# ailabspace/drl-based-mapless-crowd-navigation-with-perceived-risk

Measured on AMD Instinct MI355X. Metric: env-steps/sec @4096 envs×20 peds×360 rays; HBM GB/s vs roofline, higher is better.
Workload: dtype f64

## Files before the change

### drl-based-mapless-crowd-navigation-with-perceived-risk_amd/csrc/crowdnav_device.h

```cpp
#pragma once
#include <hip/hip_runtime.h>
#include <stdint.h>

#define CN_PI 3.14159265358979323846

typedef const __attribute__((address_space(4))) int32_t* cn_kflag;

__device__ __forceinline__ double cn_round_scaled(double x, double p, cn_kflag py2)
{
    double y = x * p;
    double r = rint(y);
    double d = y - r;
    const bool tie = fabs(d) == 0.5;
    unsigned long long any_tie = __builtin_amdgcn_ballot_w64(tie);
    asm("" : "+s"(any_tie));
    if (__builtin_expect(any_tie != 0ull, 0)) {
        if (tie) {
            double err = fma(x, p, -y);
            if (err > 0.0) r = y + 0.5;
            else if (err < 0.0) r = y - 0.5;
            else if (*py2) r = y + copysign(0.5, y);
        }
    }
    return r;
}
__device__ __forceinline__ double cn_py_round(double x, double p, cn_kflag py2) { return cn_round_scaled(x, p, py2) / p; }
__device__ __forceinline__ double cn_np_around(double x, double p) { return rint(x * p) / p; }

#define CN_INV1000 (1.0 / 1000.0)
#define CN_INV100 (1.0 / 100.0)
__device__ __forceinline__ double cn_div1000(double r)
{
    double q = r * CN_INV1000;
    return fma(fma(-q, 1000.0, r), CN_INV1000, q);
}
__device__ __forceinline__ double cn_div100(double r)
{
    double q = r * CN_INV100;
    return fma(fma(-q, 100.0, r), CN_INV100, q);
}
__device__ __forceinline__ double cn_py_round3(double x, cn_kflag py2)
{
    double r = cn_round_scaled(x, 1000.0, py2);
    return (fabs(r) < 2147483648.0) ? cn_div1000(r) : r / 1000.0;
}
__device__ __forceinline__ double cn_py_round2(double x, cn_kflag py2)
{
    double r = cn_round_scaled(x, 100.0, py2);
    return (fabs(r) < 2147483648.0) ? cn_div100(r) : r / 100.0;
}
__device__ __forceinline__ double cn_np_around3(double x)
{
    double r = rint(x * 1000.0);
    return (fabs(r) < 2147483648.0) ? cn_div1000(r) : r / 1000.0;
}
template <bool SMALL> __device__ __forceinline__ double cn_py_round3_t(double x, cn_kflag py2)
{
    if constexpr (SMALL) return cn_div1000(cn_round_scaled(x, 1000.0, py2)); else return cn_py_round3(x, py2);
}
template <bool SMALL> __device__ __forceinline__ double cn_np_around3_t(double x)
{
    if constexpr (SMALL) return cn_div1000(rint(x * 1000.0)); else return cn_np_around3(x);
}
__device__ __forceinline__ double cn_np_around2(double x)
{
    double r = rint(x * 100.0);
    return (fabs(r) < 2147483648.0) ? cn_div100(r) : r / 100.0;
}
template <bool SMALL> __device__ __forceinline__ double cn_py_round2_t(double x, cn_kflag py2)
{
    if constexpr (SMALL) return cn_div100(cn_round_scaled(x, 100.0, py2)); else return cn_py_round2(x, py2);
}
template <bool SMALL> __device__ __forceinline__ double cn_np_around2_t(double x)
{
    if constexpr (SMALL) return cn_div100(rint(x * 100.0)); else return cn_np_around2(x);
}
template <bool SMALL> __device__ __forceinline__ double cn_round_np64_2_t(double x, cn_kflag py2)
{
    const double y = x * 100.0;
    double r = rint(y);
    if (__builtin_expect(fabs(y - r) == 0.5, 0) && *py2) r = cn_round_scaled(x, 100.0, py2);
    if constexpr (SMALL) return cn_div100(r); else return (fabs(r) < 2147483648.0) ? cn_div100(r) : r / 100.0;
}

__host__ __device__ inline void cn_det_sincos(double x, double* sn, double* cs)
{
    const double two_over_pi = 6.36619772367581382433e-01;
    const double p1 = 1.57079632673412561417e+00;
    const double p2 = 6.07710050630396597660e-11;
    const double p3 = 2.02226624879595063154e-21;
    double fn = rint(x * two_over_pi);
    double r = fma(-fn, p1, x);
    r = fma(-fn, p2, r);
    r = fma(-fn, p3, r);
    double z = r * r;
    const double S1 = -1.66666666666666324348e-01, S2 = 8.33333333332248946124e-03,
                 S3 = -1.98412698298579493134e-04, S4 = 2.75573137070700676789e-06,
                 S5 = -2.50507602534068634195e-08, S6 = 1.58969099521155010221e-10;
    double ps = fma(z, S6, S5);
    ps = fma(z, ps, S4);
    ps = fma(z, ps, S3);
    ps = fma(z, ps, S2);
    ps = fma(z, ps, S1);
    double s = fma(r * z, ps, r);
    const double C1 = 4.16666666666666019037e-02, C2 = -1.38888888888741095749e-03,
                 C3 = 2.48015872894767294178e-05, C4 = -2.75573143513906633035e-07,
                 C5 = 2.08757232129817482790e-09, C6 = -1.13596475577881948265e-11;
// ... 178 lines not shown
}

__host__ __device__ inline uint64_t cn_mix64(uint64_t z)
{
    z += 0x9E3779B97F4A7C15ULL;
    z = (z ^ (z >> 30)) * 0xBF58476D1CE4E5B9ULL;
    z = (z ^ (z >> 27)) * 0x94D049BB133111EBULL;
    return z ^ (z >> 31);
}
__host__ __device__ inline double cn_rng_u01(uint64_t seed, int64_t env, uint32_t stream, uint32_t a, uint32_t b)
{
    uint64_t h = cn_mix64(seed ^ cn_mix64((uint64_t)env));
    h = cn_mix64(h ^ (((uint64_t)stream << 32) | (uint64_t)a));
    h = cn_mix64(h ^ (uint64_t)b);
    return (double)(h >> 11) * (1.0 / 9007199254740992.0);
}

__host__ __device__ inline double cn_clamp(double x, double lo, double hi) { return fmin(fmax(x, lo), hi); }

__device__ __forceinline__ double cn_iou3(double ax, double ay, double bx, double by, double half, cn_kflag py2)
{
    double axp = ax + half, axm = ax - half, ayp = ay + half, aym = ay - half;
    double bxp = bx + half, bxm = bx - half, byp = by + half, bym = by - half;
    double ix = cn_vmin(axp, bxp) - cn_vmax(axm, bxm);
    double iy = cn_vmin(ayp, byp) - cn_vmax(aym, bym);
    if (!(ix > 0.0 && iy > 0.0)) return 0.0;
    double inter = ix * iy;
    double area_a = (axp - axm) * (ayp - aym);
    double area_b = (bxp - bxm) * (byp - bym);
    double uni = area_a + area_b - inter;
    return cn_py_round3(inter / uni, py2);
}

__device__ __forceinline__ bool cn_iou3_positive(double ax, double ay, double bx, double by, double half, cn_kflag py2)
{
    double axp = ax + half, axm = ax - half, ayp = ay + half, aym = ay - half;
    double bxp = bx + half, bxm = bx - half, byp = by + half, bym = by - half;
    double ix = cn_vmin(axp, bxp) - cn_vmax(axm, bxm);
    double iy = cn_vmin(ayp, byp) - cn_vmax(aym, bym);
    if (!(ix > 0.0 && iy > 0.0)) return false;
    double inter = ix * iy;
    double area_a = (axp - axm) * (ayp - aym);
    double area_b = (bxp - bxm) * (byp - bym);
    double uni = area_a + area_b - inter;
    if (inter > 0.00075 * uni) return true;
    return cn_py_round3(inter / uni, py2) > 0.0;
}

__device__ __forceinline__ double cn_shfl_xor_d(double v, int m)
{
    int lo = __double2loint(v), hi = __double2hiint(v);
    lo = __shfl_xor(lo, m, 64);
    hi = __shfl_xor(hi, m, 64);
    return __hiloint2double(hi, lo);
}
template <int CTRL, int ROW_MASK>
__device__ __forceinline__ int cn_dpp_i(int ident, int v) { return __builtin_amdgcn_update_dpp(ident, v, CTRL, ROW_MASK, 0xf, false); }
template <int CTRL, int ROW_MASK>
__device__ __forceinline__ double cn_dpp_d(double ident, double v)
{
    int lo = __builtin_amdgcn_update_dpp(__double2loint(ident), __double2loint(v), CTRL, ROW_MASK, 0xf, false);
    int hi = __builtin_amdgcn_update_dpp(__double2hiint(ident), __double2hiint(v), CTRL, ROW_MASK, 0xf, false);
    return __hiloint2double(hi, lo);
}
template <int N> __device__ __forceinline__ int cn_row_shr_i(int ident, int v) { static_assert(N >= 1 && N <= 15, "row_shr"); return cn_dpp_i<0x110 + N, 0xf>(ident, v); }
template <int N> __device__ __forceinline__ int cn_row_shl_i(int ident, int v) { static_assert(N >= 1 && N <= 15, "row_shl"); return cn_dpp_i<0x100 + N, 0xf>(ident, v); }
#pragma clang diagnostic push
#pragma clang diagnostic ignored "-Winline-asm"
__device__ __forceinline__ unsigned long long cn_writelane_u64(unsigned long long v, unsigned long long x, int l)
{
    unsigned lo = (unsigned)v, hi = (unsigned)(v >> 32);
    const unsigned xl = __builtin_amdgcn_readfirstlane((unsigned)x), xh = __builtin_amdgcn_readfirstlane((unsigned)(x >> 32));
    const int ls = __builtin_amdgcn_readfirstlane(l);
    asm("s_mov_b32 m0, %4\n\tv_writelane_b32 %0, %2, m0\n\tv_writelane_b32 %1, %3, m0"
        : "+v"(lo), "+v"(hi) : "s"(xl), "s"(xh), "s"(ls) : "m0");
    return ((unsigned long long)hi << 32) | lo;
}
#pragma clang diagnostic pop
__device__ __forceinline__ unsigned long long cn_readlane_u64(unsigned long long v, int l)
{
    const unsigned lo = (unsigned)__builtin_amdgcn_readlane((int)(unsigned)v, l), hi = (unsigned)__builtin_amdgcn_readlane((int)(unsigned)(v >> 32), l);
    return ((unsigned long long)hi << 32) | lo;
}
#define CN_DPP_REDUCE(T, DPP, v, ident, OP)                         \
    do {                                                            \
        v = OP(v, DPP<0x111, 0xf>(ident, v));        \
        v = OP(v, DPP<0x112, 0xf>(ident, v));        \
        v = OP(v, DPP<0x114, 0xf>(ident, v));        \
        v = OP(v, DPP<0x118, 0xf>(ident, v));        \
        v = OP(v, DPP<0x142, 0xa>(ident, v));     \
        v = OP(v, DPP<0x143, 0xc>(ident, v));     \
    } while (0)
__device__ __forceinline__ double cn_lane63_d(double v)
{
    int lo = __builtin_amdgcn_readlane(__double2loint(v), 63), hi = __builtin_amdgcn_readlane(__double2hiint(v), 63);
    return __hiloint2double(hi, lo);
}
__device__ __forceinline__ double cn_wave_min_d(double v)
{
    const double id = INFINITY;
    CN_DPP_REDUCE(double, cn_dpp_d, v, id, cn_vmin);
    return cn_lane63_d(v);
}
__device__ __forceinline__ double cn_wave_max_d(double v)
{
    const double id = -INFINITY;
    CN_DPP_REDUCE(double, cn_dpp_d, v, id, cn_vmax);
    return cn_lane63_d(v);
}
__device__ __forceinline__ int cn_add_i(int a, int b) { return a + b; }
__device__ __forceinline__ int cn_wave_min_i(int v)
{
    const int id = 0x7fffffff;
    CN_DPP_REDUCE(int, cn_dpp_i, v, id, min);
    return __builtin_amdgcn_readlane(v, 63);
}
__device__ __forceinline__ int cn_wave_max_i(int v)
{
    const int id = (int)0x80000000;
    CN_DPP_REDUCE(int, cn_dpp_i, v, id, max);
    return __builtin_amdgcn_readlane(v, 63);
}
__device__ __forceinline__ int cn_wave_sum_i(int v)
{
    const int id = 0;
    CN_DPP_REDUCE(int, cn_dpp_i, v, id, cn_add_i);
    return __builtin_amdgcn_readlane(v, 63);
}
```

### drl-based-mapless-crowd-navigation-with-perceived-risk_amd/csrc/crowdnav_kernel.hip

```cpp
#include "crowdnav_device.h"
#include "crowdnav_kernel.h"

#define CN_SYNC() do { __builtin_amdgcn_fence(__ATOMIC_RELEASE, "wavefront"); __builtin_amdgcn_wave_barrier(); \
                       __builtin_amdgcn_fence(__ATOMIC_ACQUIRE, "wavefront"); } while (0)

__device__ __forceinline__ void cn_setprio_uniform(int v)
{
    if (v == 0) __builtin_amdgcn_s_setprio(0); else if (v == 1) __builtin_amdgcn_s_setprio(1);
    else if (v == 2) __builtin_amdgcn_s_setprio(2); else __builtin_amdgcn_s_setprio(3);
}
#define CN_FAIR_AT(k) do { if constexpr (FAIR) { if ((k) == 0) __builtin_amdgcn_s_setprio(3); else if ((k) == 7) __builtin_amdgcn_s_setprio(2); \
                           else if ((k) == 11) __builtin_amdgcn_s_setprio(1); else if ((k) == 15) __builtin_amdgcn_s_setprio(0); } \
                           else if constexpr (SFENCE) { if ((k) == 0 || (k) == 7 || (k) == 11 || (k) == 15) __builtin_amdgcn_s_setprio(0); } } while (0)
#ifdef CN_TIMING
#define CN_ABLATE(bit) (p->ablate & (bit))
#define CN_T(k) do { CN_FAIR_AT(k); if (p->timing && lane == 0) p->timing[(size_t)env * 32 + (k)] = (long long)__builtin_amdgcn_s_memtime(); \
                     if (((p->ablate >> 8) & 0xff) == (k) + 1 && (!((p->ablate >> 16) & 1) || (env & 3) != 0)) __builtin_amdgcn_endpgm(); } while (0)
#else
#define CN_ABLATE(bit) 0
#define CN_T(k) CN_FAIR_AT(k)
#endif

#define CN_XBAR() do { asm volatile("s_waitcnt lgkmcnt(0)\n\ts_barrier" ::: "memory"); } while (0)
struct XMail { double px, py, sy, cy, ox, oy, smin1, pad; int nnear, wall_x, wall_y, nocc, fast_assoc, k1, fe1, lb1, ns1; };
// ... 976 lines not shown
        for (int j = lane; j < nconf; j += 64) chk_set<CMP>(L, j, 0);
        CN_SYNC();
        if (nconf == 0) {
            e.ntracks = 0;
        } else {
            unsigned long long alive = 0ull;
            int cur = nt0;
            int mybj = 0; bool mymatch = false;
            for (int t0 = 0; t0 < nt0; t0 += 8) {
                const int ti = t0 + (lane >> 3);
                double best = -1.0; int bj = 0x7fffffff;
                if (ti < nt0) {
                    const double tx = TRK(CN_TF_PX, ti), ty_ = TRK(CN_TF_PY, ti);
                    for (int oj = lane & 7; oj < nconf; oj += 8) {
                        const double u = cn_iou3(tx, ty_, cfx_at<CMP>(L, oj), cfy_at<CMP>(L, oj), 0.0505, PY2);
                        if (u > best) { best = u; bj = oj; }
                    }
                }
#define CN_AM_STEP(CTRL) { const double ob = cn_dpp_d<CTRL, 0xf>(best, best); const int ojx = cn_dpp_i<CTRL, 0xf>(bj, bj); \
                           if (ob > best || (ob == best && ojx < bj)) { best = ob; bj = ojx; } }
                CN_AM_STEP(0xF5)
                CN_AM_STEP(0xEE)
                CN_AM_STEP(0x104)
#undef CN_AM_STEP
                const u64 posm = __ballot(best > 0.0);
                const int wb = __shfl(bj, (lane & 7) * 8, 64);
                if ((lane >> 3) == (t0 >> 3)) { mybj = wb; mymatch = ((posm >> (8 * (lane & 7))) & 1ull) != 0ull; }
            }
            const u64 matchm = __ballot(mymatch && lane < nt0);
            for (int i = 0; i < nt0; ++i) {
                if ((matchm >> i) & 1ull) alive |= (1ull << i);
                else if (cur > i) cur -= 1;
                else alive |= (1ull << i);
            }
            if (lane < nt0 && ((matchm >> lane) & 1ull)) {
                const int i = lane;
                double cxj = cfx_at<CMP>(L, mybj), cyj = cfy_at<CMP>(L, mybj);
                TRK(CN_TF_PX, i) = cxj; TRK(CN_TF_PY, i) = cyj; TRK(CN_TF_DIST, i) = cfd_at<CMP>(L, mybj);
                if (TRK(CN_TF_DQLEN, i) < 1.5) { TRK(CN_TF_D1X, i) = cxj; TRK(CN_TF_D1Y, i) = cyj; TRK(CN_TF_DQLEN, i) = 2.0; }
                TRK(CN_TF_T, i) = now - TRK(CN_TF_T, i);
                chk_set<CMP>(L, mybj, 1);
            }
            CN_SYNC();
            double rec[CN_TF_COUNT];
            bool mine = (lane < nt0) && ((alive >> lane) & 1ull);
            if (mine) {
#pragma unroll
                for (int f = 0; f < CN_TF_COUNT; ++f) rec[f] = TRK(f, lane);
            }
            CN_SYNC();
            if (mine) {
                int slot = __popcll(alive & ((1ull << lane) - 1ull));
#pragma unroll
                for (int f = 0; f < CN_TF_COUNT; ++f) TRK(f, slot) = rec[f];
            }
            e.ntracks = __popcll(alive);
            add_unchecked = true;
        }
    }
    CN_SYNC();
    if (add_unchecked) {
        for (int j0 = 0; j0 < nconf; j0 += 64) {
            int j = j0 + lane;
            bool want = (j < nconf) && !chk_at<CMP>(L, j) && (cft_at<CMP>(L, j) == TY_O);
            unsigned long long m = __ballot(want);
            int slot = e.ntracks + __popcll(m & ((1ull << lane) - 1ull));
            if (want) {
                if (slot < L.tcap) {
                    double cxj = cfx_at<CMP>(L, j), cyj = cfy_at<CMP>(L, j);
                    TRK(CN_TF_PX, slot) = cxj; TRK(CN_TF_PY, slot) = cyj; TRK(CN_TF_DIST, slot) = cfd_at<CMP>(L, j);
                    TRK(CN_TF_D0X, slot) = cxj; TRK(CN_TF_D0Y, slot) = cyj; TRK(CN_TF_D1X, slot) = 0.0; TRK(CN_TF_D1Y, slot) = 0.0;
                    TRK(CN_TF_T, slot) = now; TRK(CN_TF_SPEED, slot) = -1.0;
                    TRK(CN_TF_VX, slot) = 0.0; TRK(CN_TF_VY, slot) = 0.0; TRK(CN_TF_DQLEN, slot) = 1.0;
                }
            }
            int total = e.ntracks + __popcll(m);
            if (total > L.tcap) { e.status |= CN_ST_TRACK_OVERFLOW; total = L.tcap; }
            e.ntracks = total;
        }
    }
    CN_SYNC();
}

template <bool EXT, bool GT = false, bool FAIR = false, bool CMP = false, bool X2 = false, bool SF = false, bool HOIST = true, bool WIDE = false>
__device__ __forceinline__ void observe(KP p, const Poly& pg, EnvRegs& e, const Lds& L, int env, int lane, int step_counter,
                        float* obs32, float* fin32, double* obs64, int* done_out, bool have_tg = false, Trig tg = Trig{0.0, 0.0, 0.0, 0.0},
                        const int wv = 0, XMail* const mb = nullptr)
{
    constexpr bool SFENCE = SF || (CMP && !FAIR);
    static_assert(!X2 || (!EXT && !GT), "two wavefronts per environment: simulated sensors, lidar-tracker mode");
    static_assert(!WIDE || (!GT && !CMP && !X2), "the wide tracker table: lidar-tracker mode, plain layout, one wavefront");
    const bool w0 = !X2 || wv == 0;
    const int R = p->R, n = R - 1, K = p->K, D = n + 7 + 4 * K;
    const double MAXR = p->max_scan_range;
    double px = e.rx, py = e.ry;
    const double yaw = e.ryaw, v = e.rv, w = e.rw, now = e.clock;
    double distance_to_goal = 0.0, heading = 0.0, agent_vel_x = 0.0, agent_vel_y = 0.0;
    double sy = 0.0, cy = 0.0, ox = 0.0, oy = 0.0;
    const double h = p->room_half;
    int nnear = 0;
    u64 blkw = 0ull;
    bool wall_x = false, wall_y = false;
    if (w0) {
    CN_T(22);
    if (step_counter == 1) waypoint_refresh(p, pg, e, lane, px, py);
    distance_to_goal = cn_round_np64_2_t<!EXT>(dist3(px, py, e.wpx, e.wpy), PY2);
    heading = cn_py_round2_t<!EXT>(heading_to_goal(p, e, px, py, yaw), PY2);
    CN_T(23);
    if (step_counter % 5 == 0 || distance_to_goal < e.prev_dist) waypoint_refresh(p, pg, e, lane, px, py);
    CN_T(24);
    double sw_, cw_;
    if (have_tg) { sw_ = tg.sw; cw_ = tg.cw; } else cn_det_sincos_t(p->trig, w, &sw_, &cw_);
    agent_vel_x = -1.0 * (v * cw_);
    agent_vel_y = v * sw_;

    CN_T(2);
    if (have_tg) { sy = tg.sy; cy = tg.cy; } else cn_det_sincos_t(p->trig, yaw, &sy, &cy);
    ox = fma(p->lidar_offset_x, cy, px); oy = fma(p->lidar_offset_x, sy, py);
    if constexpr (X2) { if (lane == 0) { mb->px = px; mb->py = py; mb->sy = sy; mb->cy = cy; mb->ox = ox; mb->oy = oy; } }
    }
    if constexpr (X2) CN_XBAR();
    if (w0) {
    nnear = near_peds(p, L, lane, ox, oy, sy, cy, X2 ? nullptr : &blkw);
    wall_x = !(h - fabs(ox) > p->lidar_max + 1e-6);
    wall_y = !(h - fabs(oy) > p->lidar_max + 1e-6);
    if constexpr (X2) { if (lane == 0) { mb->nnear = nnear; mb->wall_x = wall_x; mb->wall_y = wall_y; } }
    }
    if constexpr (X2) {
        CN_XBAR();
        if (!w0) {
            px = mb->px; py = mb->py; sy = mb->sy; cy = mb->cy; ox = mb->ox; oy = mb->oy;
            nnear = mb->nnear; wall_x = mb->wall_x != 0; wall_y = mb->wall_y != 0;
        }
    }
    CN_T(3);
    double smin = 1e300;
    float* o32 = obs32 + (size_t)env * D;
    float* f32 = fin32 ? fin32 + (size_t)env * D : nullptr;
    double* o64 = obs64 ? obs64 + (size_t)env * D : nullptr;
    const double* const lidc = p->lidar_c; const double* const lids = p->lidar_s;
    const double* const angs = p->ang_s; const double* const angc = p->ang_c;
    short assoc_pre = 0;
    if (!GT && p->assoc_fast && lane <= p->assoc_k1 + 1) assoc_pre = p->assoc_tab[lane];
    double lmin_reg = 0.0;
    int rare_reg = 0;
    if constexpr (HOIST) {
        lmin_reg = p->lidar_min;
        rare_reg = (p->scan_f32 != 0 ? 1 : 0) | (p->lidar_min_positive ? 0 : 2);
        asm volatile("" : "+v"(lmin_reg), "+v"(rare_reg));
    }
    for (int k = X2 ? lane + 64 * wv : lane; k < R; k += X2 ? 128 : 64) {
        double lc = 0.0, ls = 0.0, tS = 0.0, tC = 0.0;
        if (!EXT) { lc = cn_ldg(lidc, (unsigned)k); ls = cn_ldg(lids, (unsigned)k); }
        if (!GT) { tS = cn_ldg(angs, (unsigned)(R - 1 - k)); tC = cn_ldg(angc, (unsigned)(R - 1 - k)); }
        const double t = cast_ray<EXT>(p, L, env, k, ox, oy, sy, cy, nnear, wall_x, wall_y, lc, ls, X2 ? nullptr : &blkw, HOIST ? &lmin_reg : nullptr, HOIST);
        if (k >= 1) {
            const unsigned j = (unsigned)(R - 1 - k);
            double r = t;
            double sc;
            if constexpr (EXT) {
                if (isinf(r) && r > 0) sc = MAXR;
                else if (r != r) sc = 0.0;
                else if (r == 0.0) sc = MAXR;
                else if (r > MAXR) sc = MAXR;
                else sc = r;
            } else {
                sc = cn_vmin(r, MAXR);
                const int rare = HOIST ? __builtin_amdgcn_readfirstlane(rare_reg) : (p->lidar_min_positive ? 0 : 2);
                if (__builtin_expect(rare != 0, 0)) {
                    if (rare & 1) r = (double)(float)r;
                    sc = cn_vmin(r, MAXR);
                    if ((rare & 2) && r == 0.0) sc = MAXR;
                }
            }
            smin = cn_vmin(smin, sc);
            if constexpr (!GT) {
            const double sa = fma(tS, cy, -(tC * sy)), ca = fma(tC, cy, tS * sy);
            pt_set<CMP>(L, j, (int)cn_round_scaled(px + (sc * ca), 1000.0, PY2), (int)cn_round_scaled(py + (sc * sa) * -1.0, 1000.0, PY2));
            L.dmil[j] = (unsigned short)(int)cn_round_scaled(sc, 1000.0, PY2);
            }
            double so = cn_np_around3_t<!EXT>(sc);
            cn_stg(o32, j, (float)so);
            if (f32) cn_stg(f32, j, (float)so);
            if (o64) cn_stg(o64, j, so);
        }
    }
    CN_T(4);
    bool too_close = __ballot(smin < p->min_scan_range) != 0ull;
    CN_SYNC();
    if constexpr (X2) {
        if (!w0 && lane == 0) mb->smin1 = too_close ? -1.0 : 1e300;
        CN_XBAR();
        if (w0) too_close = too_close || (mb->smin1 < 0.0);
    }

    if (w0 && step_counter == 0) {
        if (!EXT && p->bb_spawn_valid && px == p->spawn_x && py == p->spawn_y && yaw == p->spawn_yaw) e.bb = p->bb_spawn;
        else e.bb = bbox_size(p, L.stage, lane, n, px, py, yaw);
        double qx = cn_py_round3_t<!EXT>(px, PY2), qy = cn_py_round3_t<!EXT>(py, PY2);
        if (e.dq_len < 2) { if (e.dq_len == 0) { e.dq0x = qx; e.dq0y = qy; } else { e.dq1x = qx; e.dq1y = qy; } e.dq_len += 1; }
        else { e.dq0x = e.dq1x; e.dq0y = e.dq1y; e.dq1x = qx; e.dq1y = qy; }
    }

    CN_T(5);
    int ego_hit = 0;
    double* const T = WIDE ? L.gtrk : L.trk;
    double* const CPV = WIDE ? L.gcpv : L.cpv;
    if constexpr (!GT) {
    const int W = (n + 63) >> 6;
#define WORD(id, q) L.w64[__mul24((id), L.wstride) + (q)]
#define BIT(id, i) ((WORD(id, (i) >> 6) >> ((i) & 63)) & 1ull)
#define PX(i) cn_div1000((double)ptx_at<CMP>(L, (i)))
#define PY(i) cn_div1000((double)pty_at<CMP>(L, (i)))
#define GNONE 0x7fffffff
    unsigned short* occlist = L.srcidx;
    int nocc = 0;
    u64 occraw = 0ull;
    if (w0)
    for (int q = 0; q < W; ++q) {
        const int i = lane + 64 * q;
        const bool oc = (i < n) && (L.dmil[i] != 600);
        if (i < n) L.gq[i] = GNONE;
        const u64 bo = __ballot(oc);
        if (oc) occlist[nocc + __popcll(bo & ((1ull << lane) - 1ull))] = (unsigned short)i;
        occraw = cn_writelane_u64(occraw, bo, q);
        nocc += __popcll(bo);
    }
    if (w0 && lane < W) { WORD(M_NONE, lane) = ~0ull; WORD(M_ZERO, lane) = 0ull; WORD(M_EQ, lane) = 0ull; WORD(M_NNONE, lane) = 0ull; WORD(M_NZERO, lane) = 0ull; }
    CN_SYNC();
    if constexpr (X2) {
        if (w0 && lane == 0) mb->nocc = nocc;
        CN_XBAR();
        if (!w0) nocc = mb->nocc;
    }
    for (int c0 = 0; c0 < nocc; c0 += 128) {
        const int ca = X2 ? c0 + 64 * wv + lane : c0 + lane, cb = X2 ? nocc : ca + 64;
        const bool two = !X2 && c0 + 64 < nocc;
        const bool va = ca < nocc, vb = cb < nocc;
        const int ia = va ? (int)occlist[ca] : 0, ib = vb ? (int)occlist[cb] : 0;
        const int ja = (ia == n - 1) ? 0 : ia + 1, jb = (ib == n - 1) ? 0 : ib + 1;
        const int xai = ptx_at<CMP>(L, ia), yai = pty_at<CMP>(L, ia), xaj = ptx_at<CMP>(L, ja), yaj = pty_at<CMP>(L, ja);
        int xbi = 0, ybi = 0, xbj = 0, ybj = 0;
        if (two) { xbi = ptx_at<CMP>(L, ib); ybi = pty_at<CMP>(L, ib); xbj = ptx_at<CMP>(L, jb); ybj = pty_at<CMP>(L, jb); }
        const double dya = cn_div1000((double)yai) - cn_div1000((double)yaj);
        const double qa = (dya == 0) ? 0.0 : cn_div(cn_div1000((double)xai) - cn_div1000((double)xaj), dya);
        if (va) L.gq[ia] = (int)cn_round_scaled(qa, 1000.0, PY2);
        if (two) {
            const double dyb = cn_div1000((double)ybi) - cn_div1000((double)ybj);
            const double qb = (dyb == 0) ? 0.0 : cn_div(cn_div1000((double)xbi) - cn_div1000((double)xbj), dyb);
            if (vb) L.gq[ib] = (int)cn_round_scaled(qb, 1000.0, PY2);
        }
    }
    int lastnn = -1;
    if (nocc > 0) {
        lastnn = occlist[nocc - 1];
        if (lastnn == n - 1) lastnn = (nocc > 1) ? (int)occlist[nocc - 2] : -1;
    }
    CN_SYNC();
    if constexpr (X2) CN_XBAR();
#define CHG(a_, b_) (((a_) == GNONE || (b_) == GNONE) ? CN_NAN : fabs(cn_div1000((double)(a_)) - cn_div1000((double)(b_))))
    double clast = CN_NAN;
    if (L.gq[n - 1] != GNONE && lastnn >= 0) clast = CHG(L.gq[lastnn], L.gq[lastnn + 1]);
// ... 356 lines not shown
#undef GNONE
    e.nconf = nconf;
    CN_SYNC();

    int n_obst = 0;
    for (int j = lane; j < nconf; j += 64) {
        if (cft_at<CMP>(L, j) == TY_O) { n_obst += 1; if (cfd_at<CMP>(L, j) < 0.140) ego_hit = 1; }
    }
    n_obst = cn_wave_sum_i(n_obst);
    ego_hit = cn_wave_max_i(ego_hit);
    if (n_obst > 0) e.obst_steps += 1;

    CN_T(13);
    if constexpr (WIDE) tracker_stage_wide(p, e, L, T, lane, nconf, now);
    else tracker_stage<CMP>(p, e, L, T, lane, nconf, now);
    } else {
        const int P_ = p->P;
        const double r_ = p->ped_radius, lim_ = p->lidar_max + r_, lim2_ = lim_ * lim_;
        int nt_ = 0;
        u64 hitm = 0ull;
        for (int i0 = 0; i0 < P_; i0 += 64) {
            const int i = i0 + lane;
            bool inr = false, seg = false, blocked = false;
            double cx = 0.0, cyy = 0.0, wx = 0.0, wy = 0.0, len2 = 0.0;
            if (i < P_) {
                cx = L.ped[2 * i]; cyy = L.ped[2 * i + 1];
                const double ocx = cx - ox, ocy = cyy - oy;
                const double dd2 = fma(ocx, ocx, ocy * ocy);
                inr = dd2 <= lim2_;
                if (inr) {
                    const double dd = cn_sqrt(dd2);
                    if (dd > r_) {
                        seg = true;
                        const double k_ = (dd - r_) / dd;
                        wx = k_ * ocx; wy = k_ * ocy;
                        len2 = fma(wx, wx, wy * wy);
                    }
                }
            }
            for (int j0 = 0; j0 < P_; j0 += 64) {
                const int jl = j0 + lane;
                bool jin = false;
                if (jl < P_) { const double qx = L.ped[2 * jl] - ox, qy = L.ped[2 * jl + 1] - oy; jin = fma(qx, qx, qy * qy) <= lim2_; }
                u64 jm = __ballot(jin);
                while (jm) {
                    const int j = j0 + __builtin_ctzll(jm);
                    jm &= jm - 1ull;
                    const double qx = L.ped[2 * j] - ox, qy = L.ped[2 * j + 1] - oy;
                    if (seg && j != i) {
                        double tau = (len2 > 0.0) ? fma(qx, wx, qy * wy) / len2 : 0.0;
                        tau = fmin(fmax(tau, 0.0), 1.0);
                        const double ex = fma(tau, wx, -qx), ey = fma(tau, wy, -qy);
                        if (fma(ex, ex, ey * ey) < r_ * r_) blocked = true;
                    }
                }
            }
            const bool vis = inr && !blocked;
            const u64 vm = __ballot(vis);
            const int slot = nt_ + __popcll(vm & ((1ull << lane) - 1ull));
            bool close_ = false;
            if (vis && slot < L.tcap) {
                const double dx = cx - px, dy = cyy - py;
                const double dp = cn_sqrt(fma(dx, dx, dy * dy));
                double sx_ = cx, sy_ = cyy;
                if (dp > 0.0) { sx_ = cx - r_ * (dx / dp); sy_ = cyy - r_ * (dy / dp); }
                const double dist = cn_py_round3(dp - r_, PY2);
                const double vx = L.pedv[2 * i], vy = L.pedv[2 * i + 1];
                TRK(CN_TF_PX, slot) = cn_py_round3(sx_, PY2); TRK(CN_TF_PY, slot) = cn_py_round3(sy_, PY2); TRK(CN_TF_DIST, slot) = dist;
                TRK(CN_TF_D0X, slot) = 0.0; TRK(CN_TF_D0Y, slot) = 0.0; TRK(CN_TF_D1X, slot) = 0.0; TRK(CN_TF_D1Y, slot) = 0.0;
                TRK(CN_TF_T, slot) = (double)i; TRK(CN_TF_SPEED, slot) = cn_sqrt(fma(vx, vx, vy * vy));
                TRK(CN_TF_VX, slot) = -vx; TRK(CN_TF_VY, slot) = -vy; TRK(CN_TF_DQLEN, slot) = 0.0;
                close_ = dist < 0.140;
            }
            hitm |= __ballot(close_);
            nt_ += __popcll(vm);
        }
        if (nt_ > L.tcap) { e.status |= CN_ST_TRACK_OVERFLOW; nt_ = L.tcap; }
        e.ntracks = nt_; e.nconf = nt_;
        if (nt_ > 0) e.obst_steps += 1;
        ego_hit = hitm != 0ull;
        CN_SYNC();
    }
    CN_T(14);
    if constexpr (WIDE) {
        for (int it = lane; it < e.ntracks; it += 64) {
            if (TRK(CN_TF_DQLEN, it) > 1.5) {
                double dc = cn_hypot(TRK(CN_TF_D0Y, it) - TRK(CN_TF_D1Y, it), TRK(CN_TF_D0X, it) - TRK(CN_TF_D1X, it));
                TRK(CN_TF_SPEED, it) = cn_div_z(dc, TRK(CN_TF_T, it));
            }
        }
    } else
    if (lane < e.ntracks && TRK(CN_TF_DQLEN, lane) > 1.5) {
        double dc = cn_hypot(TRK(CN_TF_D0Y, lane) - TRK(CN_TF_D1Y, lane), TRK(CN_TF_D0X, lane) - TRK(CN_TF_D1X, lane));
        TRK(CN_TF_SPEED, lane) = cn_div_z(dc, TRK(CN_TF_T, lane));
    }
    CN_TSYNC();

    for (int i = lane; i < 4 * K; i += 64) {
        int c = i & 3;
        L.tail[7 + i] = (c == 0) ? px : (c == 1 ? py : 0.0);
    }
    if (lane < K) L.kidx[lane] = -1;
    e.nent = 0;
    CN_SYNC();

    CN_T(15);
    if (e.dq_len == 2 && !(CN_ABLATE(8))) {
        const double ts = e.ts;
        if (ts == 0.0) e.status |= CN_ST_DT_ZERO;
        const int nt = e.ntracks;
        double vx_ = cn_div_z(e.dq1x - e.dq0x, ts), vy_ = cn_div_z(e.dq1y - e.dq0y, ts);
        double agent_vel = cn_sqrt(vx_ * vx_ + vy_ * vy_);
        double obstacle_vel = (nt == 0) ? 0.0 : TRK(CN_TF_SPEED, 0);
        if constexpr (WIDE) {
            for (int it = lane; it < nt; it += 64)
                if (TRK(CN_TF_DQLEN, it) > 1.5) {
                    double chx = TRK(CN_TF_D0X, it) - TRK(CN_TF_D1X, it), chy = TRK(CN_TF_D0Y, it) - TRK(CN_TF_D1Y, it);
                    TRK(CN_TF_VX, it) = cn_div_z(chx, ts); TRK(CN_TF_VY, it) = cn_div_z(chy, ts);
                }
            CN_WIDE_SYNC();
        } else
        if (!GT && lane < nt && TRK(CN_TF_DQLEN, lane) > 1.5) {
            double chx = TRK(CN_TF_D0X, lane) - TRK(CN_TF_D1X, lane), chy = TRK(CN_TF_D0Y, lane) - TRK(CN_TF_D1Y, lane);
            TRK(CN_TF_VX, lane) = cn_div_z(chx, ts); TRK(CN_TF_VY, lane) = cn_div_z(chy, ts);
        }
        double vo_x = e.dq1x, vo_y = e.dq1y;
        if (nt > 0) {
            int l = nt - 1;
            double chx = 0.0, chy = 0.0;
            if (GT) { chx = TRK(CN_TF_VX, l) * ts; chy = TRK(CN_TF_VY, l) * ts; }
            else if (TRK(CN_TF_DQLEN, l) > 1.5) { chx = TRK(CN_TF_D0X, l) - TRK(CN_TF_D1X, l); chy = TRK(CN_TF_D0Y, l) - TRK(CN_TF_D1Y, l); }
            vo_x = e.dq1x + chx; vo_y = e.dq1y + chy;
        }
        CN_SYNC();
        const double a0x = e.dq0x, a0y = e.dq0y;
        double gradient = (vo_y == 0.0) ? 0.0 : cn_div(vo_x - a0x, vo_y) - a0y;
        double bb0 = a0x - (gradient * a0y);
        int hi = (int)ceil(a0x + 3.5), lo = (int)floor(a0x - 3.5);
        double ego_max = 0.0;
        const double rv = agent_vel - obstacle_vel;
        const int hcap = min(p->max_conf, 64);
        double* const hitp = L.cfx;
        for (int c0 = 0; c0 < nt; c0 += hcap) {
            const int c1 = min(nt, c0 + hcap);
            u64 nearm = 0, hasm = 0;
            for (int i = c0; i < c1; ++i) {
                const int r_ = i - c0;
                if ((r_ & 7) == 0) {
                    const int ti = i + (lane >> 3), x2l = hi - (lane & 7);
                    bool nearc = false;
                    if (ti < c1 && x2l > lo) {
                        const double ctx = TRK(CN_TF_PX, ti), cty = TRK(CN_TF_PY, ti);
                        const double y2l = ((double)x2l * gradient) + bb0;
                        const double ex = (double)x2l - a0x, ey = y2l - a0y, fx = ctx - a0x, fy = cty - a0y;
                        const double ee = ex * ex + ey * ey, ff = fx * fx + fy * fy, num = fx * ex + fy * ey;
                        const double rr2 = 0.178 * 0.178 * 1.000001;
                        bool far_;
                        if (num <= 0.0) far_ = ff > rr2;
                        else if (num >= ee) far_ = (fx - ex) * (fx - ex) + (fy - ey) * (fy - ey) > rr2;
                        else far_ = (ff - rr2) * ee > num * num * 1.000001;
                        nearc = !far_;
                    }
                    nearm = __ballot(nearc);
                }
                unsigned cand = (unsigned)((nearm >> (8 * (r_ & 7))) & 0xffull);
                if (p->geos_untyped_empty) cand &= 1u;
                if (!cand) continue;
                const double tx = TRK(CN_TF_PX, i), ty_ = TRK(CN_TF_PY, i);
                while (cand) {
                    const int c = __builtin_ctz(cand);
                    cand &= cand - 1u;
                    const int x2 = hi - c;
                    double y2 = ((double)x2 * gradient) + bb0;
                    double hx = 0.0, hy = 0.0;
                    unsigned long long m = ring_segment(pg, lane, tx, ty_, 0.178, a0x, a0y, (double)x2, y2, &hx, &hy);
                    int cnt = __popcll(m);
                    if (cnt == 0) continue;
                    if (cnt == 1) break;
                    const int l1 = __ffsll((long long)m) - 1;
                    const int l2 = __ffsll((long long)(m & (m - 1ull))) - 1;
                    if (lane == l1) { hitp[r_] = hx; hitp[hcap + r_] = hy; }
                    if (lane == l2) { hitp[2 * hcap + r_] = hx; hitp[3 * hcap + r_] = hy; }
                    hasm |= 1ull << r_;
                    break;
                }
            }
            CN_SYNC();
            {
                const int i = c0 + lane;
                double ego = 0.0;
                bool ttc0 = false;
                if (i < c1) {
                    const double td = TRK(CN_TF_DIST, i);
                    const double gcp = (td > p->max_scan_range) ? 0.0 : cn_div(p->max_scan_range - td, p->max_scan_range - p->min_scan_range);
                    double cpv;
                    if ((hasm >> lane) & 1ull) {
                        const double d1 = cn_hypot(a0x - hitp[lane], a0y - hitp[hcap + lane]);
                        const double d2 = cn_hypot(a0x - hitp[2 * hcap + lane], a0y - hitp[3 * hcap + lane]);
                        const double dcp = cn_vmin(d1, d2);
                        if (rv == 0) { cpv = 1.0 * gcp; ego = 0.0; }
                        else {
                            double ttc = EXT ? dcp / rv : cn_div(dcp, rv);
                            if (ttc == 0.0) { ttc0 = true; ego = 1.0; }
                            else ego = fmin(1.0, EXT ? 0.15 / ttc : cn_div(0.15, ttc));
                            cpv = 0.5 * ego + 0.5 * gcp;
                        }
                    } else { ego = 0.0; cpv = 0.5 * 0.0 + 0.5 * gcp; }
                    CPV[i] = cpv;
                }
                if (__ballot(ttc0) != 0ull) e.status |= CN_ST_TTC_ZERO;
                const double first = lane_d(ego, 0);
                const bool rest = (i < c1) && !(c0 == 0 && lane == 0) && (ego == ego);
                const double mrest = cn_wave_max_d(rest ? ego : -INFINITY);
                if (c0 == 0) ego_max = first;
                if (mrest > ego_max) ego_max = mrest;
            }
            CN_SYNC();
        }
        e.nent = nt;
        CN_TSYNC();
        double cprob_new = 0.0, ego_new = 0.0;
        if (nt != 0) {
            ego_new = ego_max;
            int first = nt > K ? nt - K : 0;
            if constexpr (WIDE) {
                for (int c0 = 0; c0 < nt; c0 += 64) {
                    const int it = c0 + lane;
                    int rank = -1; double mycp = 0.0;
                    if (it < nt) {
                        mycp = CPV[it];
                        rank = 0;
                        for (int j = 0; j < nt; ++j) {
                            const double c = CPV[j];
                            rank += (c > mycp) || (c == mycp && j < it);
                        }
                        if (rank >= first) {
                            const int kk = rank - first;
                            L.tail[7 + 4 * kk + 0] = TRK(CN_TF_PX, it); L.tail[7 + 4 * kk + 1] = TRK(CN_TF_PY, it);
                            L.tail[7 + 4 * kk + 2] = TRK(CN_TF_VX, it); L.tail[7 + 4 * kk + 3] = TRK(CN_TF_VY, it);
                            L.kidx[kk] = it;
                        }
                    }
                    const u64 mf = __ballot(rank == first);
                    if (mf) cprob_new = bcast_d(mycp, __ffsll((long long)mf) - 1);
                }
            } else {
            int rank = -1; double mycp = 0.0;
            if (lane < nt) mycp = L.cpv[lane];
            if (nt <= 8) {
                const int ti = lane >> 3, tj = lane & 7;
                bool beats = false;
                if (ti < nt && tj < nt) { const double ci = L.cpv[ti], cj = L.cpv[tj]; beats = (cj > ci) || (cj == ci && tj < ti); }
                const u64 bm = __ballot(beats);
                if (lane < nt) rank = __popc((unsigned)(bm >> (8 * lane)) & 0xffu);
            } else if (lane < nt) {
                rank = 0;
                for (int j = 0; j < nt; ++j) {
                    double c = L.cpv[j];
                    rank += (c > mycp) || (c == mycp && j < lane);
                }
            }
            if (lane < nt) {
                if (rank >= first) {
                    int kk = rank - first;
                    L.tail[7 + 4 * kk + 0] = TRK(CN_TF_PX, lane); L.tail[7 + 4 * kk + 1] = TRK(CN_TF_PY, lane);
                    L.tail[7 + 4 * kk + 2] = TRK(CN_TF_VX, lane); L.tail[7 + 4 * kk + 3] = TRK(CN_TF_VY, lane);
                    L.kidx[kk] = GT ? (int)TRK(CN_TF_T, lane) : lane;
                }
            }
            unsigned long long mf = __ballot(rank == first);
            cprob_new = bcast_d(mycp, __ffsll((long long)mf) - 1);
            }
        }
        e.cprob = cprob_new; e.ego = ego_new;
        e.dq0x = e.dq1x; e.dq0y = e.dq1y; e.dq_len = 1;
        if constexpr (WIDE) { for (int it = lane; it < nt; it += 64) TRK(CN_TF_T, it) = now; }
        else
        if (!GT && lane < nt) TRK(CN_TF_T, lane) = now;
    }
    CN_T(16);
    if (ego_hit) e.ego_viol += 1;
    if (e.ego > 0.4) e.social_viol += 1;
// ... 637 lines not shown
                CN_SYNC();
                int d1 = 0;
                observe<EXT, GT, FAIR, CMP, true, SFENCE>(p, pg, e, L, env, lane, 0, io_obs(), do_reset ? nullptr : p->final_obs, p->obs_f64, &d1, false,
                                                  Trig{0.0, 0.0, 0.0, 0.0}, 1, mb);
                return;
            }
        }
        int sc = 0;
        float* fin = nullptr;
        Trig trig = Trig{0.0, 0.0, 0.0, 0.0}; bool have_trig = false;
        double rs1 = 0.0, rc1 = 0.0, rs2 = 0.0, rc2 = 0.0;
        bool ph_pre = true, ph_obs = true, ph_rew = true;
        if constexpr (EXT) {
            if (p->ext_phase) { ph_pre = p->ext_phase & CN_PHASE_PRE; ph_obs = p->ext_phase & CN_PHASE_GET_STATE; ph_rew = p->ext_phase & CN_PHASE_REWARD; }
        }
        if (!do_reset) {
            if (ph_pre) e.ep_step += 1;
            sc = p->step_counter ? p->step_counter[env] : e.ep_step;
            double deq_x, deq_y, end_timestep;
            if (!ext) {
                double v, w;
                if (act_pre) { v = (double)a0_pre; w = (double)a1_pre; }
                else { const float* const ain = act_here ? act_here : io_action() + 2 * (size_t)env; v = (double)ain[0]; w = (double)ain[1]; }
                const double t0 = e.clock;
                if constexpr (SIM == 3) { e.cv = v; e.cw = w; } else { e.rv = v; e.rw = w; }
                e.clock += cn_div1000((double)p->dt_ms);
                if constexpr (SIM != 0) sim_advance_ticks<SIM>(p, e, env, lane, L.ped, pedv, (double*)smem, p->dt_ms);
                else {
                if constexpr (LAYOUT == 0) { step_trig(p, e, lane, rs1, rc1, rs2, rc2, trig); have_trig = true; }
                CN_T(27);
                if constexpr (!X2)
                ped_advance<SHAPE == 360>(p, env, lane, L.ped, pedv, e.crowd_ms, e.crowd_ms + p->dt_ms + p->scan_latency_ms, p->dt_ms);
                CN_T(28);
                e.crowd_ms += p->dt_ms + p->scan_latency_ms;
                if (have_trig) robot_advance_sc(p, e, p->dt_ms, rs1, rc1); else robot_advance(p, e, p->dt_ms);
                }
                CN_T(20);
                end_timestep = e.clock - t0;
                if constexpr (LAYOUT == 2)
                    end_timestep = 0.0 + ((cn_div1000((double)p->dt_ms) - 0.0) + 0.1);
                deq_x = e.rx; deq_y = e.ry;
                fin = p->final_obs;
            } else {
                deq_x = od[6]; deq_y = od[7]; end_timestep = od[8];
            }
            if (ph_pre) {
            double qx = cn_py_round3_t<!EXT>(deq_x, PY2), qy = cn_py_round3_t<!EXT>(deq_y, PY2);
            if (e.dq_len == 0) { e.dq0x = qx; e.dq0y = qy; e.dq_len = 1; }
            else if (e.dq_len == 1) { e.dq1x = qx; e.dq1y = qy; e.dq_len = 2; }
            else { e.dq0x = e.dq1x; e.dq0y = e.dq1y; e.dq1x = qx; e.dq1y = qy; }
            e.ts = end_timestep;
            }
            if (!ext) {
                e.clock += cn_div1000((double)p->scan_latency_ms);
                if constexpr (SIM != 0) sim_advance_ticks<SIM>(p, e, env, lane, L.ped, pedv, (double*)smem, p->scan_latency_ms);
                else if (have_trig) robot_advance_sc(p, e, p->scan_latency_ms, rs2, rc2); else robot_advance(p, e, p->scan_latency_ms);
                CN_T(21);
            }
        } else {
            if (!ext) {
                e.rx = p->spawn_x; e.ry = p->spawn_y; e.ryaw = p->spawn_yaw; e.rv = 0.0; e.rw = 0.0; e.cv = 0.0; e.cw = 0.0;
                for (int i = lane; i < 2 * P; i += 64) { L.ped[i] = gped_init[i]; pedv[i] = 0.0; }
                CN_SYNC();
                e.clock += cn_div1000((double)p->scan_latency_ms);
                if constexpr (SIM != 0) sim_advance_ticks<SIM>(p, e, env, lane, L.ped, pedv, (double*)smem, p->scan_latency_ms);
                else sim_advance(p, e, env, lane, L.ped, pedv, p->scan_latency_ms);
            }
            if constexpr (LAYOUT == 1) {
                e.prev_dist = dist3(e.rx, e.ry, p->goal_x, p->goal_y);
                e.prev_head = orig_heading(p, e.rx, e.ry, e.ryaw);
            } else if constexpr (LAYOUT == 2) {
                e.prev_dist = rw_distance(p, e.rx, e.ry);
                e.prev_head = rw_heading(p, e.rx, e.ry, e.ryaw);
            } else {
            e.prev_dist = dist3(e.rx, e.ry, e.wpx, e.wpy);
            e.prev_head = heading_to_goal(p, e, e.rx, e.ry, e.ryaw);
            }
        }
        pedv_save();
        CN_SYNC();
        if (ph_obs) {
            if constexpr (LAYOUT == 1) observe_original<EXT>(p, e, L, env, lane, sc, io_obs(), fin, p->obs_f64, &done);
            else if constexpr (LAYOUT == 2) observe_realworld<EXT>(p, pg, e, L, RQ, env, lane, sc, io_obs(), fin, p->obs_f64, &done);
            else observe<EXT, GT, FAIR, CMP, X2, SFENCE, !(FUSED && SHAPE == 720), WIDE>(p, pg, e, L, env, lane, sc, io_obs(), fin, p->obs_f64, &done, have_trig, trig, 0, mb);
        } else if constexpr (EXT) {
            const int D_ = (LAYOUT == 1) ? n + 4 : (LAYOUT == 2 ? n + 11 : n + 7 + 4 * K);
            if (lane < 4) {
                const int src = (LAYOUT == 1) ? n + lane : n + (lane & 1);
                L.tail[lane] = p->obs_f64 ? p->obs_f64[(size_t)env * D_ + src] : (double)p->obs[(size_t)env * D_ + src];
            }
            done = io_done()[env] ? 1 : 0;
            e.nconf = __builtin_amdgcn_readlane(cold_i, CN_SI_NCONF); e.nent = __builtin_amdgcn_readlane(cold_i, CN_SI_NENTRIES);
            CN_SYNC();
        }
        cold_settle();
        if (!do_reset && !ph_rew) {
            if (lane == 0) io_done()[env] = (uint8_t)done;
            if (ph_obs && io_topk() && lane < K) io_topk()[(size_t)env * K + lane] = LAYOUT != 0 ? -1 : L.kidx[lane];
        } else
        if (!do_reset) {
            double r;
            if constexpr (LAYOUT == 1) r = compute_reward_original(p, e, L, done);
            else if constexpr (LAYOUT == 2) r = compute_reward_realworld(p, e, L, done);
            else r = compute_reward(p, pg, e, L, lane, done);
            e.ep_ret += r;
            if (lane == 0) {
                io_reward()[env] = (float)r;
                io_done()[env] = (uint8_t)done;
            }
            if (ph_obs && io_topk() && lane < K) io_topk()[(size_t)env * K + lane] = LAYOUT != 0 ? -1 : L.kidx[lane];
            if (done) {
                if (!ext) { if constexpr (SIM == 3) { e.cv = 0.0; e.cw = 0.0; } else { e.rv = 0.0; e.rw = 0.0; } }
                e.last_ret = e.ep_ret;
                e.episodes += 1;
                e.pending = !ext && (p->auto_reset == 2);
                if (lane == 0) {
                    sd[CN_SD_LAST_EGO_VIOL] = (double)e.ego_viol; sd[CN_SD_LAST_SOCIAL_VIOL] = (double)e.social_viol;
                    sd[CN_SD_LAST_OBST_STEPS] = (double)e.obst_steps; sd[CN_SD_LAST_EP_STEPS] = (double)e.ep_step;
                }
            }
        } else {
            e.social_viol = 0; e.ego_viol = 0; e.obst_steps = 0;
            if (!ext) {
                e.clock += cn_div1000((double)p->settle_ms);
                pedv_restore();
                if constexpr (SIM != 0) sim_advance_ticks<SIM>(p, e, env, lane, L.ped, pedv, (double*)smem, p->settle_ms);
                else sim_advance(p, e, env, lane, L.ped, pedv, p->settle_ms);
                CN_SYNC();
                pedv_save();
            }
            e.done = 0;
            e.ep_step = 0; e.ep_ret = 0.0; e.pending = 0;
        }
        CN_SYNC();
    } else {
    bool need_reset = (p->mode == CN_MODE_RESET || p->mode == CN_MODE_EXT_RESET);
    if (p->mode == CN_MODE_STEP && p->auto_reset == 2 && e.pending) {
        need_reset = true;
        e.pending = 0;
        if (lane == 0) { io_reward()[env] = 0.0f; io_done()[env] = 0; }
        if (io_topk() && lane < K) io_topk()[(size_t)env * K + lane] = -1;
    } else if (p->mode == CN_MODE_STEP || p->mode == CN_MODE_EXT_STEP) {
        e.ep_step += 1;
        const int sc = p->step_counter ? p->step_counter[env] : e.ep_step;
        double deq_x, deq_y, end_timestep;
        if (!ext) {
            const double v = (double)io_action()[2 * env], w = (double)io_action()[2 * env + 1];
            const double t0 = e.clock;
            if constexpr (SIM == 3) { e.cv = v; e.cw = w; } else { e.rv = v; e.rw = w; }
            e.clock += cn_div1000((double)p->dt_ms);
            if constexpr (SIM != 0) sim_advance_ticks<SIM>(p, e, env, lane, L.ped, pedv, (double*)smem, p->dt_ms);
            else {
            ped_advance(p, env, lane, L.ped, pedv, e.crowd_ms, e.crowd_ms + p->dt_ms + p->scan_latency_ms, p->dt_ms);
            e.crowd_ms += p->dt_ms + p->scan_latency_ms;
            robot_advance(p, e, p->dt_ms);
            }
            end_timestep = e.clock - t0;
                if constexpr (LAYOUT == 2)
                    end_timestep = 0.0 + ((cn_div1000((double)p->dt_ms) - 0.0) + 0.1);
            deq_x = e.rx; deq_y = e.ry;
        } else {
            deq_x = od[6]; deq_y = od[7]; end_timestep = od[8];
        }
        {
            double qx = cn_py_round3(deq_x, PY2), qy = cn_py_round3(deq_y, PY2);
            if (e.dq_len == 0) { e.dq0x = qx; e.dq0y = qy; e.dq_len = 1; }
            else if (e.dq_len == 1) { e.dq1x = qx; e.dq1y = qy; e.dq_len = 2; }
// ... 668 lines not shown
```

Before: 111.4 million.

## Share wave lanes across collision-point distances and track speed hypot passes

Adds a SHARE template mode, on for fixed-shape single-wavefront plain-layout builds. In it the two hit-point distance hypots per track are split across the two wave halves and combined with a permlane32 swap and min, and the idle upper lanes compute track speeds in the same pass. It also merges the three tie-checked roundings of lidar hit points into one ballot. The aim is fewer serial double-precision hypot/div passes and ballots per step, at the cost of more complex lane-mapping logic that only applies under narrow conditions (dq_len==2, at most 21 tracks).

```diff
diff --git a/drl-based-mapless-crowd-navigation-with-perceived-risk_amd/csrc/crowdnav_device.h b/drl-based-mapless-crowd-navigation-with-perceived-risk_amd/csrc/crowdnav_device.h
--- a/drl-based-mapless-crowd-navigation-with-perceived-risk_amd/csrc/crowdnav_device.h
+++ b/drl-based-mapless-crowd-navigation-with-perceived-risk_amd/csrc/crowdnav_device.h
@@ -23,6 +23,27 @@
         }
     }
     return r;
+}
+__device__ __forceinline__ void cn_round_scaled3(double x0, double x1, double x2, double p, cn_kflag py2, double* r0, double* r1, double* r2)
+{
+    const double y0 = x0 * p, y1 = x1 * p, y2 = x2 * p;
+    double q0 = rint(y0), q1 = rint(y1), q2 = rint(y2);
+    const bool t0 = fabs(y0 - q0) == 0.5, t1 = fabs(y1 - q1) == 0.5, t2 = fabs(y2 - q2) == 0.5;
+    unsigned long long any_tie = __builtin_amdgcn_ballot_w64(t0 || t1 || t2);
+    asm("" : "+s"(any_tie));
+    if (__builtin_expect(any_tie != 0ull, 0)) {
+        auto fix = [&](double x, double y, double r) {
+            const double err = fma(x, p, -y);
+            if (err > 0.0) r = y + 0.5;
+            else if (err < 0.0) r = y - 0.5;
+            else if (*py2) r = y + copysign(0.5, y);
+            return r;
+        };
+        if (t0) q0 = fix(x0, y0, q0);
+        if (t1) q1 = fix(x1, y1, q1);
+        if (t2) q2 = fix(x2, y2, q2);
+    }
+    *r0 = q0; *r1 = q1; *r2 = q2;
 }
 __device__ __forceinline__ double cn_py_round(double x, double p, cn_kflag py2) { return cn_round_scaled(x, p, py2) / p; }
 __device__ __forceinline__ double cn_np_around(double x, double p) { return rint(x * p) / p; }
@@ -367,7 +388,14 @@
     const unsigned lo = (unsigned)__builtin_amdgcn_readlane((int)(unsigned)v, l), hi = (unsigned)__builtin_amdgcn_readlane((int)(unsigned)(v >> 32), l);
     return ((unsigned long long)hi << 32) | lo;
 }
-#define CN_DPP_REDUCE(T, DPP, v, ident, OP)                         \
+__device__ __forceinline__ double cn_min_halves(double v)
+{
+    const unsigned lo = (unsigned)__double2loint(v), hi = (unsigned)__double2hiint(v);
+    const auto l = __builtin_amdgcn_permlane32_swap(lo, lo, false, false);
+    const auto h = __builtin_amdgcn_permlane32_swap(hi, hi, false, false);
+    return cn_vmin(__hiloint2double((int)h[0], (int)l[0]), __hiloint2double((int)h[1], (int)l[1]));
+}
+#define CN_DPP_REDUCE(T, DPP, v, ident, OP)                       \
     do {                                                            \
         v = OP(v, DPP<0x111, 0xf>(ident, v));        \
         v = OP(v, DPP<0x112, 0xf>(ident, v));        \
diff --git a/drl-based-mapless-crowd-navigation-with-perceived-risk_amd/csrc/crowdnav_kernel.hip b/drl-based-mapless-crowd-navigation-with-perceived-risk_amd/csrc/crowdnav_kernel.hip
--- a/drl-based-mapless-crowd-navigation-with-perceived-risk_amd/csrc/crowdnav_kernel.hip
+++ b/drl-based-mapless-crowd-navigation-with-perceived-risk_amd/csrc/crowdnav_kernel.hip
@@ -1082,7 +1082,7 @@
     CN_SYNC();
 }
 
-template <bool EXT, bool GT = false, bool FAIR = false, bool CMP = false, bool X2 = false, bool SF = false, bool HOIST = true, bool WIDE = false>
+template <bool EXT, bool GT = false, bool FAIR = false, bool CMP = false, bool X2 = false, bool SF = false, bool HOIST = true, bool WIDE = false, bool SHARE = false>
 __device__ __forceinline__ void observe(KP p, const Poly& pg, EnvRegs& e, const Lds& L, int env, int lane, int step_counter,
                         float* obs32, float* fin32, double* obs64, int* done_out, bool have_tg = false, Trig tg = Trig{0.0, 0.0, 0.0, 0.0},
                         const int wv = 0, XMail* const mb = nullptr)
@@ -1090,6 +1090,7 @@
     constexpr bool SFENCE = SF || (CMP && !FAIR);
     static_assert(!X2 || (!EXT && !GT), "two wavefronts per environment: simulated sensors, lidar-tracker mode");
     static_assert(!WIDE || (!GT && !CMP && !X2), "the wide tracker table: lidar-tracker mode, plain layout, one wavefront");
+    static_assert(!SHARE || (!WIDE && !X2), "shared passes: one wavefront per environment, the LDS track table");
     const bool w0 = !X2 || wv == 0;
     const int R = p->R, n = R - 1, K = p->K, D = n + 7 + 4 * K;
     const double MAXR = p->max_scan_range;
@@ -1176,8 +1177,15 @@
             smin = cn_vmin(smin, sc);
             if constexpr (!GT) {
             const double sa = fma(tS, cy, -(tC * sy)), ca = fma(tC, cy, tS * sy);
+            if constexpr (SHARE) {
+                double ex_, ey_, er_;
+                cn_round_scaled3(px + (sc * ca), py + (sc * sa) * -1.0, sc, 1000.0, PY2, &ex_, &ey_, &er_);
+                pt_set<CMP>(L, j, (int)ex_, (int)ey_);
+                L.dmil[j] = (unsigned short)(int)er_;
+            } else {
             pt_set<CMP>(L, j, (int)cn_round_scaled(px + (sc * ca), 1000.0, PY2), (int)cn_round_scaled(py + (sc * sa) * -1.0, 1000.0, PY2));
             L.dmil[j] = (unsigned short)(int)cn_round_scaled(sc, 1000.0, PY2);
+            }
             }
             double so = cn_np_around3_t<!EXT>(sc);
             cn_stg(o32, j, (float)so);
@@ -1700,6 +1708,8 @@
         CN_SYNC();
     }
     CN_T(14);
+    const int hcap = min(p->max_conf, 64);
+    const bool dc_shared = SHARE && e.dq_len == 2 && !(CN_ABLATE(8)) && e.ntracks >= 1 && e.ntracks <= 21 && hcap >= 32;
     if constexpr (WIDE) {
         for (int it = lane; it < e.ntracks; it += 64) {
             if (TRK(CN_TF_DQLEN, it) > 1.5) {
@@ -1707,6 +1717,8 @@
                 TRK(CN_TF_SPEED, it) = cn_div_z(dc, TRK(CN_TF_T, it));
             }
         }
+    } else
+    if (dc_shared) {
     } else
     if (lane < e.ntracks && TRK(CN_TF_DQLEN, lane) > 1.5) {
         double dc = cn_hypot(TRK(CN_TF_D0Y, lane) - TRK(CN_TF_D1Y, lane), TRK(CN_TF_D0X, lane) - TRK(CN_TF_D1X, lane));
@@ -1756,8 +1768,7 @@
         double bb0 = a0x - (gradient * a0y);
         int hi = (int)ceil(a0x + 3.5), lo = (int)floor(a0x - 3.5);
         double ego_max = 0.0;
-        const double rv = agent_vel - obstacle_vel;
-        const int hcap = min(p->max_conf, 64);
+        double rv = agent_vel - obstacle_vel;
         double* const hitp = L.cfx;
         for (int c0 = 0; c0 < nt; c0 += hcap) {
             const int c1 = min(nt, c0 + hcap);
@@ -1804,6 +1815,20 @@
                 }
             }
             CN_SYNC();
+            const bool share_d = SHARE && c1 - c0 <= 32 && hcap >= 32;
+            double dcp_sh = 0.0;
+            if (share_d && (hasm != 0ull || dc_shared)) {
+                const int tl = lane & 31, up = lane >> 5;
+                double hx_ = a0x - hitp[2 * up * hcap + tl], hy_ = a0y - hitp[(2 * up + 1) * hcap + tl];
+                const int dt_ = tl - 21 + 11 * up;
+                const bool dcl = dc_shared && tl >= 21 && dt_ < nt && TRK(CN_TF_DQLEN, dt_) > 1.5;
+                if (dcl) { hx_ = TRK(CN_TF_D0Y, dt_) - TRK(CN_TF_D1Y, dt_); hy_ = TRK(CN_TF_D0X, dt_) - TRK(CN_TF_D1X, dt_); }
+                const double hd = cn_hypot(hx_, hy_);
+                double sp = 0.0;
+                if (dcl) { sp = cn_div_z(hd, TRK(CN_TF_T, dt_)); TRK(CN_TF_SPEED, dt_) = sp; }
+                if (dc_shared && TRK(CN_TF_DQLEN, 0) > 1.5) rv = agent_vel - lane_d(sp, 21);
+                dcp_sh = cn_min_halves(hd);
+            }
             {
                 const int i = c0 + lane;
                 double ego = 0.0;
@@ -1813,9 +1838,13 @@
                     const double gcp = (td > p->max_scan_range) ? 0.0 : cn_div(p->max_scan_range - td, p->max_scan_range - p->min_scan_range);
                     double cpv;
                     if ((hasm >> lane) & 1ull) {
+                        double dcp;
+                        if (share_d) dcp = dcp_sh;
+                        else {
                         const double d1 = cn_hypot(a0x - hitp[lane], a0y - hitp[hcap + lane]);
                         const double d2 = cn_hypot(a0x - hitp[2 * hcap + lane], a0y - hitp[3 * hcap + lane]);
-                        const double dcp = cn_vmin(d1, d2);
+                        dcp = cn_vmin(d1, d2);
+                        }
                         if (rv == 0) { cpv = 1.0 * gcp; ego = 0.0; }
                         else {
                             double ttc = EXT ? dcp / rv : cn_div(dcp, rv);
@@ -2619,7 +2648,7 @@
         if (ph_obs) {
             if constexpr (LAYOUT == 1) observe_original<EXT>(p, e, L, env, lane, sc, io_obs(), fin, p->obs_f64, &done);
             else if constexpr (LAYOUT == 2) observe_realworld<EXT>(p, pg, e, L, RQ, env, lane, sc, io_obs(), fin, p->obs_f64, &done);
-            else observe<EXT, GT, FAIR, CMP, X2, SFENCE, !(FUSED && SHAPE == 720), WIDE>(p, pg, e, L, env, lane, sc, io_obs(), fin, p->obs_f64, &done, have_trig, trig, 0, mb);
+            else observe<EXT, GT, FAIR, CMP, X2, SFENCE, !(FUSED && SHAPE == 720), WIDE, SHAPE != 0 && !X2 && !WIDE && !GT>(p, pg, e, L, env, lane, sc, io_obs(), fin, p->obs_f64, &done, have_trig, trig, 0, mb);
         } else if constexpr (EXT) {
             const int D_ = (LAYOUT == 1) ? n + 4 : (LAYOUT == 2 ? n + 11 : n + 7 + 4 * K);
             if (lane < 4) {
```

Result: no change. 112.1 million, median of 5 (+0.7%).
